# ekzhu/datasketch

Hardware: AMD Instinct MI355X
Metric: MinHash signatures/sec (1M sets x 256 tokens, num_perm=128) (higher is better)
Workload: dtype u64

## Files before the change

datasketch_amd/csrc/mhx_api.hip:

```cpp
#include <algorithm>
#include <cmath>
#include <condition_variable>
#include <cstdlib>
#include <cstring>
#include <mutex>
#include <new>
#include <system_error>
#include <thread>
#include <vector>

#include "mhx_internal.h"

namespace mhx {

static thread_local std::string g_last_error;

void set_error(const char *fmt, ...) {
    char buf[1024];
    va_list ap;
    va_start(ap, fmt);
    vsnprintf(buf, sizeof(buf), fmt, ap);
    va_end(ap);
    g_last_error = buf;
}
// ... 186 lines not shown
        (void)hipStreamSynchronize(stream);
        (void)mhx::dev_free(d_redo);
        d_redo = nullptr;
        redo_capacity = 0;
    }
    const int64_t cap = std::max<int64_t>(n_sets + n_sets / 4, 1024);
    hipError_t e = mhx::dev_malloc(reinterpret_cast<void **>(&d_redo), (size_t)cap + 64);
    if (e != hipSuccess) {
        d_redo = nullptr;
        return fail(MHX_ERR_OOM, "redo flag allocation of %lld bytes failed: %s", (long long)cap, hipGetErrorString(e));
    }
    redo_capacity = cap;
    return MHX_OK;
}

int mhx_ctx::ensure_work() {
    if (d_work) return MHX_OK;
    hipError_t e = mhx::dev_malloc(reinterpret_cast<void **>(&d_work), mhx::kWorkBytes);
    if (e != hipSuccess) {
        d_work = nullptr;
        return fail(MHX_ERR_OOM, "work counter allocation failed: %s", hipGetErrorString(e));
    }
    MHX_HIP_CHECK(hipMemsetAsync(d_work, 0, mhx::kWorkBytes, stream));
    return MHX_OK;
}

extern "C" {

const char *mhx_last_error(void) { return mhx::g_last_error.c_str(); }

const char *mhx_version(void) { return "mhx 0.1.0 (gfx950)"; }

int mhx_device_count(int *count) {
    if (!count) return fail(MHX_ERR_INVALID, "count is NULL");
    int n = 0;
    hipError_t e = hipGetDeviceCount(&n);
    if (e != hipSuccess) {
        (void)hipGetLastError();
        *count = 0;
        return MHX_OK;
    }
    *count = n;
    return MHX_OK;
}

int mhx_ctx_create(int device, mhx_ctx **out) {
// ... 12 lines not shown
    ctx->device = device;
    ctx->num_cus = prop.multiProcessorCount;
    ctx->lds_per_block = (int64_t)prop.sharedMemPerBlock;
    ctx->hbm_bytes = (int64_t)prop.totalGlobalMem;
    snprintf(ctx->name, sizeof(ctx->name), "%s (%s)", prop.name, prop.gcnArchName);
    hipError_t e = hipStreamCreateWithFlags(&ctx->stream, hipStreamNonBlocking);
    if (e != hipSuccess) {
        delete ctx;
        return fail(MHX_ERR_HIP, "hipStreamCreate failed: %s", hipGetErrorString(e));
    }
    *out = ctx;
    return MHX_OK;
}

int mhx_ctx_destroy(mhx_ctx *ctx) {
    if (!ctx) return MHX_OK;
    (void)hipSetDevice(ctx->device);
    (void)hipStreamSynchronize(ctx->stream);
    for (int i = 0; i < 5; ++i)
        if (ctx->scratch[i]) (void)mhx::dev_free(ctx->scratch[i]);
    if (ctx->d_stats) (void)mhx::dev_free(ctx->d_stats);
    if (ctx->d_redo) (void)mhx::dev_free(ctx->d_redo);
    if (ctx->d_work) (void)mhx::dev_free(ctx->d_work);
    if (ctx->copy_in) (void)hipStreamDestroy(ctx->copy_in);
    if (ctx->copy_out) (void)hipStreamDestroy(ctx->copy_out);
    (void)hipStreamDestroy(ctx->stream);
    delete ctx;
    return MHX_OK;
}

int mhx_ctx_synchronize(mhx_ctx *ctx) {
    if (!ctx) return fail(MHX_ERR_INVALID, "ctx is NULL");
    MHX_GUARD(ctx);
    MHX_HIP_CHECK(hipStreamSynchronize(ctx->stream));
    return MHX_OK;
}

int mhx_ctx_release_scratch(mhx_ctx *ctx) {
    if (!ctx) return fail(MHX_ERR_INVALID, "ctx is NULL");
    MHX_GUARD(ctx);
    if (int rc = ctx->activate()) return rc;
    MHX_HIP_CHECK(hipStreamSynchronize(ctx->stream));
    for (int i = 0; i < 5; ++i) {
        if (ctx->scratch[i]) MHX_HIP_CHECK(mhx::dev_free(ctx->scratch[i]));
        ctx->scratch[i] = nullptr;
        ctx->scratch_bytes[i] = 0;
// ... 5 lines not shown
    }
    return MHX_OK;
}

int mhx_ctx_device_info(mhx_ctx *ctx, char *name, int name_len, int *cus, int64_t *hbm_bytes) {
    if (!ctx) return fail(MHX_ERR_INVALID, "ctx is NULL");
    MHX_GUARD(ctx);
    if (name && name_len > 0) {
        strncpy(name, ctx->name, (size_t)name_len - 1);
        name[name_len - 1] = 0;
    }
    if (cus) *cus = ctx->num_cus;
    if (hbm_bytes) *hbm_bytes = ctx->hbm_bytes;
    return MHX_OK;
}

int mhx_ctx_set_option(mhx_ctx *ctx, const char *key, int64_t value) {
    if (!ctx || !key) return fail(MHX_ERR_INVALID, "ctx/key is NULL");
    MHX_GUARD(ctx);
    if (!strcmp(key, "minhash.path")) ctx->opt_minhash_path = value;
    else if (!strcmp(key, "minhash.split")) ctx->opt_minhash_split = value;
    else if (!strcmp(key, "minhash.packed")) ctx->opt_minhash_packed = value;
    else if (!strcmp(key, "minhash.ties")) ctx->opt_minhash_ties = value;
    else if (!strcmp(key, "minhash.p3")) ctx->opt_minhash_p3 = value;
    else if (!strcmp(key, "minhash.share")) ctx->opt_minhash_share = value;
    else if (!strcmp(key, "minhash.adapt")) ctx->opt_minhash_adapt = value;
    else if (!strcmp(key, "blocks_per_cu")) ctx->opt_blocks_per_cu = value;
    else if (!strcmp(key, "minhash.alias")) ctx->opt_minhash_alias = value;
    else if (!strcmp(key, "minhash.prefetch")) ctx->opt_minhash_prefetch = value;
    else if (!strcmp(key, "weighted.path")) ctx->opt_weighted_path = value;
    else if (!strcmp(key, "weighted.direct")) ctx->opt_weighted_direct = value;
    else if (!strcmp(key, "weighted.split")) ctx->opt_weighted_split = value;
    else if (!strcmp(key, "weighted.tail")) ctx->opt_weighted_tail = value;
    else if (!strcmp(key, "weighted.debug")) ctx->opt_weighted_debug = value;
    else if (!strcmp(key, "weighted.kernel")) ctx->opt_weighted_kernel = value;
    else if (!strcmp(key, "weighted.plan")) ctx->opt_weighted_plan = value;
    else if (!strcmp(key, "weighted.rescue")) ctx->opt_weighted_rescue = value;
    else if (!strcmp(key, "weighted.min_dim")) ctx->opt_weighted_min_dim = value;
    else if (!strcmp(key, "host.chunk_bytes")) ctx->opt_host_chunk_bytes = value;
    else if (!strcmp(key, "lsh.sort_bits")) ctx->opt_lsh_sort_bits = value;
    else if (!strcmp(key, "lsh.gather")) ctx->opt_lsh_gather = value;
    else if (!strcmp(key, "lsh.sort")) ctx->opt_lsh_sort = value;
    else if (!strcmp(key, "lsh.levels")) ctx->opt_lsh_levels = value;
    else if (!strcmp(key, "lsh.chunk")) ctx->opt_lsh_chunk = value;
    else if (!strcmp(key, "lsh.team")) ctx->opt_lsh_team = value;
    else if (!strcmp(key, "lsh.bigbins")) ctx->opt_lsh_bigbins = value;
    else if (!strcmp(key, "pack.fused")) ctx->opt_pack_fused = value;
    else if (!strcmp(key, "weighted.refill")) ctx->opt_weighted_refill = value;
    else if (!strcmp(key, "lsh.prehash")) ctx->opt_lsh_prehash = value;
    else if (!strcmp(key, "lsh.merge_items")) {
        if (value != 0 && value != 8 && value != 16) return fail(MHX_ERR_INVALID, "lsh.merge_items must be 0, 8 or 16");
        ctx->opt_lsh_merge_items = value;
    }
    else return fail(MHX_ERR_INVALID, "unknown option '%s'", key);
    return MHX_OK;
}

int mhx_ctx_minhash_mode(mhx_ctx *ctx, int reset, int *mode) {
    if (!ctx) return fail(MHX_ERR_INVALID, "ctx is NULL");
    MHX_GUARD(ctx);
    if (int rc = ctx->activate()) return rc;
    if (int rc = ctx->ensure_work()) return rc;
    unsigned int word = 0;
    MHX_HIP_CHECK(hipMemcpyAsync(&word, ctx->d_work + 8, sizeof(word), hipMemcpyDeviceToHost, ctx->stream));
    MHX_HIP_CHECK(hipStreamSynchronize(ctx->stream));
    if (mode) *mode = (int)word;
    if (reset) MHX_HIP_CHECK(hipMemsetAsync(ctx->d_work + 8, 0, sizeof(word), ctx->stream));
    return MHX_OK;
}

int mhx_ctx_minhash_flags(mhx_ctx *ctx, int64_t n_sets, uint8_t *flags) {
    if (!ctx) return fail(MHX_ERR_INVALID, "ctx is NULL");
    MHX_GUARD(ctx);
    if (int rc = ctx->activate()) return rc;
    MHX_REQUIRE(n_sets >= 0 && (flags || n_sets == 0), "NULL flags");
    if (ctx->redo_sets != n_sets || (n_sets > 0 && !ctx->d_redo))
        return fail(MHX_ERR_INVALID, "the last MinHash call on this context kept flags for %lld sets, not %lld (one huge set split over waves and "
                    "minhash.path != 0 keep none)", (long long)ctx->redo_sets, (long long)n_sets);
    MHX_HIP_CHECK(hipStreamSynchronize(ctx->stream));
    if (n_sets > 0) MHX_HIP_CHECK(hipMemcpy(flags, ctx->d_redo, (size_t)n_sets, hipMemcpyDeviceToHost));
    return MHX_OK;
}

int mhx_ctx_counters(mhx_ctx *ctx, int enable, uint64_t out[MHX_NUM_COUNTERS]) {
    if (!ctx) return fail(MHX_ERR_INVALID, "ctx is NULL");
    MHX_GUARD(ctx);
    if (int rc = ctx->activate()) return rc;
    MHX_HIP_CHECK(hipStreamSynchronize(ctx->stream));
    if (out) {
        for (int i = 0; i < MHX_NUM_COUNTERS; ++i) out[i] = 0;
// ... 1618 lines not shown
```

datasketch_amd/csrc/mhx_internal.h:

```cpp
#pragma once

#include <hip/hip_runtime.h>

#include <cstdarg>
#include <cstdint>
#include <cstdio>
#include <mutex>
#include <string>
#include <unordered_map>

#include "mhx.h"

namespace mhx {

void set_error(const char *fmt, ...);
int fail(int code, const char *fmt, ...);
void forgive();

#define MHX_HIP_CHECK(expr)                                                                      \
    do {                                                                                         \
        hipError_t _e = (expr);                                                                  \
        if (_e != hipSuccess) {                                                                  \
            return ::mhx::fail(_e == hipErrorOutOfMemory ? MHX_ERR_OOM : MHX_ERR_HIP,            \
                               "%s failed: %s (%s:%d)", #expr, hipGetErrorString(_e), __FILE__,  \
                               __LINE__);                                                        \
        }                                                                                        \
    } while (0)

constexpr int kSigDigests = 2;
constexpr int kSigDigestsBM = 3;

constexpr unsigned int kPairListCap = 16384;
constexpr size_t kWorkBytes = 64 + sizeof(unsigned int) * kPairListCap;

#define MHX_GUARD(ctxp) std::lock_guard<std::recursive_mutex> _mhx_guard((ctxp)->mu)

#define MHX_REQUIRE(cond, ...)                                       \
    do {                                                             \
        if (!(cond)) return ::mhx::fail(MHX_ERR_INVALID, __VA_ARGS__); \
    } while (0)

hipError_t dev_malloc(void **p, size_t bytes, bool caller = false);
hipError_t dev_free(void *p);
bool guard_mode();

}

struct mhx_ctx {
    std::recursive_mutex mu;
    int device = 0;
    hipStream_t stream = nullptr;
    int num_cus = 0;
    int64_t lds_per_block = 64 << 10;
    int64_t hbm_bytes = 0;
    char name[128] = {0};
    void *scratch[5] = {nullptr, nullptr, nullptr, nullptr, nullptr};
    size_t scratch_bytes[5] = {0, 0, 0, 0, 0};
    int64_t opt_minhash_path = 0;
    int64_t opt_minhash_packed = 0;
    int64_t opt_minhash_adapt = 0;
    int64_t opt_minhash_share = 0;
    int64_t opt_minhash_p3 = 0;
    int64_t opt_minhash_ties = 0;
    int64_t opt_minhash_split = 0;
    int64_t opt_blocks_per_cu = 0;
    int64_t opt_minhash_prefetch = 1;
    int64_t opt_minhash_alias = -1;
    int64_t opt_weighted_path = 0;
    int64_t opt_weighted_min_dim = 0;
    int64_t opt_weighted_rescue = 0;
    int64_t opt_weighted_plan = 0;
    int64_t opt_weighted_kernel = 0;
    int64_t opt_weighted_debug = 0;
    int64_t opt_weighted_split = 0;
    int64_t opt_weighted_tail = 0;
    int64_t opt_weighted_direct = 0;
    int64_t opt_lsh_sort = 0;
    int64_t opt_lsh_gather = 0;
    int64_t opt_lsh_sort_bits = 0;
    int64_t opt_lsh_prehash = 0;
    int64_t opt_lsh_chunk = 0;
    int64_t opt_lsh_bigbins = 0;
    int64_t opt_lsh_team = 0;
    int64_t opt_lsh_merge_items = 0;
    int64_t opt_lsh_levels = 0;
    int64_t opt_pack_fused = 0;
    int64_t opt_weighted_refill = 0;
    int64_t opt_host_chunk_bytes = 0;

    hipStream_t copy_in = nullptr;
    hipStream_t copy_out = nullptr;
    int ensure_copy_streams();

    unsigned long long *d_stats = nullptr;
    uint8_t *d_redo = nullptr;
    int64_t redo_capacity = 0;
    int64_t redo_sets = 0;
    int ensure_redo(int64_t n_sets);
    unsigned int *d_work = nullptr;
    int ensure_work();

    int ensure_scratch(int slot, size_t bytes);
    int activate() const;
};

struct mhx_perm {
    mhx_ctx *ctx = nullptr;
    int32_t num_perm = 0;
    uint64_t *d_a = nullptr;
    uint64_t *d_b = nullptr;
};

struct mhx_wgen {
    mhx_ctx *ctx = nullptr;
    int32_t sample_size = 0;
    int32_t dim = 0;
    float *d_params = nullptr;
    int32_t s_pad = 0;
    bool table_fast = false;
    float *d_aos = nullptr;
    float *d_walk_a = nullptr;
    uint32_t *d_walk_c = nullptr;
// ... 76 lines not shown
```

datasketch_amd/csrc/minhash_kernels.hip:

```cpp
#include <type_traits>

#include "mhx_internal.h"

namespace mhx {
namespace {

constexpr uint64_t kMersenne = (1ull << 61) - 1;
constexpr uint32_t kMaxHash = 0xFFFFFFFFu;
constexpr int kWave = 64;

struct BulkArgs {
    const void *hv;
    const int64_t *offsets;
    int64_t fixed_len;
    int64_t n_sets;
    const uint64_t *a;
    const uint64_t *b;
    int32_t num_perm;
    int32_t path;
    unsigned long long *stats;
    uint8_t *redo;
    int32_t redo_match;
    unsigned int *sieve_hint;
    unsigned int *mode_word;
    unsigned int *pair_count;
    unsigned int *pair_list;
    int32_t prefetch;
    int32_t ties;
    int32_t share_last;
    int64_t alias_mask;
    const uint64_t *init;
    int64_t init_stride;
    void *out;
};

__device__ __forceinline__ void mad_narrow(uint32_t h, uint32_t a_lo, uint32_t a_hi, uint64_t b,
                                           uint32_t &s_lo, uint32_t &s_hi) {
    const uint64_t s0 = (uint64_t)h * a_lo + b;
    s_lo = (uint32_t)s0;
    s_hi = (uint32_t)(s0 >> 32) + h * a_hi;
}

__device__ __forceinline__ void mad_wide(uint32_t h_lo, uint32_t h_hi, uint32_t a_lo, uint32_t a_hi,
                                         uint64_t b, uint32_t &s_lo, uint32_t &s_hi) {
    const uint64_t s0 = (uint64_t)h_lo * a_lo + b;
    s_lo = (uint32_t)s0;
    s_hi = (uint32_t)(s0 >> 32) + h_lo * a_hi + h_hi * a_lo;
// ... 694 lines not shown
        const int r = args.num_perm - (kbase + (P - 1) * kWave);
        span = r > 16 ? 32u : r > 8 ? 16u : r > 4 ? 8u : 4u;
    }
    sp.span = span;
#pragma unroll
    for (int p = 0; p < P; ++p) {
        const bool shared = SHARE && P >= 3 && p == P - 1;
        const int k = kbase + p * kWave + (shared ? lane & (int)(span - 1) : lane);
        const bool holds = k < args.num_perm;
        kidx[p] = holds && !(shared && lane >= (int)span) ? k : -1;
        const uint64_t a = holds ? args.a[k] : 0;
        pm.a_lo[p] = (uint32_t)a;
        pm.a_hi[p] = (uint32_t)(a >> 32);
        pm.b[p] = holds ? args.b[k] : 0;
        pm_biased.a_lo[p] = pm.a_lo[p];
        pm_biased.a_hi[p] = pm.a_hi[p];
        pm_biased.b[p] = pm.b[p] + 1;
        sp.a_lo[p] = pm.a_lo[p];
        sp.b8[p] = pm.b[p] + 8;
        sp.active[p] = kidx[p] >= 0;
    }
}

enum { MODE_SIEVE = 0, MODE_FULL = 1, MODE_DEDUP = 2, MODE_SIEVE_TIES = 3 };
enum { SHAPE_GENERAL = 0, SHAPE_PLAIN = 1, SHAPE_PLAIN_FIXED = 2, SHAPE_PLAIN_FIXED_ROWS = 3 };

template <int P, typename TokT, typename OutT, int MODE, int SHAPE, bool SHARE = false>
__global__ __launch_bounds__(256) void minhash_bulk_kernel(const BulkArgs args_in) {
    BulkArgs args = args_in;
    constexpr bool kSieve = MODE == MODE_SIEVE || MODE == MODE_SIEVE_TIES;
    if (kSieve && args.mode_word) {
        const unsigned int want_ties = *as_const(args.mode_word);
        if ((want_ties == 1u) != (MODE == MODE_SIEVE_TIES)) return;
    }
    if (MODE == MODE_FULL && args.mode_word && args.sieve_hint && blockIdx.x == 0 && threadIdx.x == 0) {
        const unsigned int t = __builtin_nontemporal_load(args.sieve_hint), f = __builtin_nontemporal_load(args.sieve_hint + 1);
        const unsigned int g = __builtin_nontemporal_load(args.sieve_hint + 2), m = *args.mode_word;
        const unsigned int tt = __builtin_nontemporal_load(args.sieve_hint + 3), tf = __builtin_nontemporal_load(args.sieve_hint + 5);
        if (t >= 64u) {
            const bool defeated = 4u * f > t;
            const bool heavy = m == 1u ? 5u * g > t : (tt >= 64u ? 5u * tf > tt : m == 2u);
            *args.mode_word = !defeated ? 0u : heavy ? 2u : 1u;
        }
    }
    if (SHAPE != SHAPE_GENERAL) {
        args.init = nullptr;
        args.init_stride = 0;
        args.stats = nullptr;
        args.alias_mask = -1;
    }
    if (SHAPE == SHAPE_PLAIN_FIXED || SHAPE == SHAPE_PLAIN_FIXED_ROWS) args.offsets = nullptr;
    const int lane = threadIdx.x & (kWave - 1);
    const int wave = __builtin_amdgcn_readfirstlane(threadIdx.x >> 6);
    const int waves_per_block = blockDim.x >> 6;
    const int kchunks = (args.num_perm + kWave * P - 1) / (kWave * P);
    constexpr int kLdsPerWave = MODE == MODE_DEDUP ? kDedupWordsPerWave : kStageWordsPerWave;
    __shared__ __attribute__((aligned(16))) uint32_t stage[4 * kLdsPerWave];
    uint32_t *lds = stage + wave * kLdsPerWave;
    Perms<P> pm, pm_biased;
    SievePerms<P> sp;
    int kidx[P];
    if (kSieve || MODE == MODE_DEDUP) load_perms<P, SHARE>(args, 0, lane, pm, pm_biased, sp, kidx);

    const TokT MHX_CONST_AS *hv = as_const(static_cast<const TokT *>(args.hv));
    const TokT *hv_vec = static_cast<const TokT *>(args.hv);
    const int64_t MHX_CONST_AS *offsets = as_const(args.offsets);
    OutT *__restrict__ out = static_cast<OutT *>(args.out);
    const int64_t stride = (int64_t)gridDim.x * waves_per_block;
    const bool flagged_only = !kSieve && args.redo != nullptr;
    unsigned int listed_n = 0;
    bool listed = false;
    if (MODE == MODE_FULL && flagged_only && args.pair_list) {
        listed_n = *as_const(args.pair_count);
        listed = listed_n <= kPairListCap;
    }
    const int64_t n_items = listed ? (int64_t)listed_n : flagged_only ? (args.n_sets + kWave - 1) / kWave * waves_per_block : args.n_sets;
    SieveBackoff backoff;
    TiesBackoff ties;
    int tried = 0, failed = 0, left = 0;
    if (MODE == MODE_SIEVE && args.sieve_hint) {
        const unsigned int t = __builtin_nontemporal_load(args.sieve_hint), f = __builtin_nontemporal_load(args.sieve_hint + 1);
        if (t >= 64u && 2u * f > t) {
            backoff.skip = 63;
            backoff.gap = 64;
            backoff.streak = 2;
        }
    }
    if (MODE == MODE_FULL && listed) {
        uint32_t *comb = stage;
        for (int64_t it = blockIdx.x; it < (int64_t)listed_n; it += gridDim.x) {
            const int64_t set = (int64_t)as_const(args.pair_list)[it];
            const int64_t beg = args.offsets ? offsets[set] : set * args.fixed_len;
            const int64_t end = args.offsets ? offsets[set + 1] : beg + args.fixed_len;
            const int64_t share = (end - beg + 31) / 32 * 8;
            const int64_t wbeg = min(end, beg + wave * share), wend = min(end, wbeg + share);
            for (int kc = 0; kc < kchunks; ++kc) {
                uint32_t mine[P];
#pragma unroll
                for (int p = 0; p < P; ++p) mine[p] = kMaxHash;
                if (wend > wbeg) {
                    const Minima<P> m = full_minima<P, TokT>(hv_vec, wbeg, wend, args.a, args.b, args.num_perm, kc * (kWave * P),
                                                             args.path == 1, args.stats);
#pragma unroll
                    for (int p = 0; p < P; ++p) mine[p] = m.v[p];
                }
#pragma unroll
                for (int p = 0; p < P; ++p) comb[(wave * P + p) * kWave + lane] = mine[p];
                __syncthreads();
                if (wave == 0) {
#pragma unroll
                    for (int p = 0; p < P; ++p) {
                        const int k = kc * (kWave * P) + p * kWave + lane;
                        if (k >= args.num_perm) continue;
                        uint32_t r = mine[p];
#pragma unroll
                        for (int w = 1; w < 4; ++w) r = min(r, comb[(w * P + p) * kWave + lane]);
                        uint64_t v = r;
                        if (args.init) {
                            const uint64_t iv = args.init[set * args.init_stride + k];
                            v = end > beg ? (uint64_t)min((iv >> 32) ? kMaxHash : (uint32_t)iv, r) : iv;
                        }
                        if (sizeof(OutT) == 4) v = v > kMaxHash ? kMaxHash : v;
                        out[set * args.num_perm + k] = (OutT)v;
                    }
                }
                __syncthreads();
            }
        }
        return;
    }
    for (int64_t item0 = (int64_t)blockIdx.x * waves_per_block + wave; item0 < n_items; item0 += stride) {
      const int64_t item = flagged_only ? item0 / waves_per_block : item0;
      unsigned long long todo = 1;
      if (flagged_only && !listed) {
          const int64_t cand = item * kWave + lane;
          const bool mine = (lane % waves_per_block) == (int)(item0 % waves_per_block);
          todo = __ballot(mine && cand < args.n_sets && args.redo[cand] == (uint8_t)args.redo_match);
      }
      while (todo) {
        const int bit = __builtin_ctzll(todo);
        todo &= todo - 1;
        const int64_t set = listed ? (int64_t)as_const(args.pair_list)[item0] : flagged_only ? item * kWave + bit : item;
        int64_t beg, end;
        if (args.offsets) {
            beg = offsets[set];
            end = offsets[set + 1];
        } else {
            beg = (args.alias_mask >= 0 ? (set & args.alias_mask) : set) * args.fixed_len;
            end = beg + args.fixed_len;
        }
        uint32_t warm = 0;
        {
            const int64_t nset = listed ? args.n_sets : flagged_only ? (todo ? item * kWave + __builtin_ctzll(todo) : args.n_sets) : item + stride;
            const bool skipping_on = MODE == MODE_SIEVE && backoff.skip > 1;
            if (args.prefetch && nset < args.n_sets && !skipping_on) {
                const int64_t nbeg = args.offsets ? offsets[nset] : nset * args.fixed_len;
                const int64_t nend = args.offsets ? offsets[nset + 1] : nbeg + args.fixed_len;
                const int64_t off = (int64_t)lane * 128;
                if (off < (nend - nbeg) * (int64_t)sizeof(TokT))
                    warm = *reinterpret_cast<const volatile uint32_t *>(reinterpret_cast<const char *>(args.hv) +
                                                                         nbeg * (int64_t)sizeof(TokT) + off);
            }
        }
        bool defer = false;
        if (MODE == MODE_SIEVE && end > beg && backoff.skip > 0) {
            --backoff.skip;
            defer = true;
        }
        for (int kc = 0; kc < kchunks && !defer; ++kc) {
            uint32_t res[P];
            if (kSieve) {
                if (kchunks > 1) load_perms<P, SHARE>(args, kc * (kWave * P), lane, pm, pm_biased, sp, kidx);
                if (end > beg) {
                    bool tied = false;
                    defer = sieve_minima<P, TokT, SHAPE != SHAPE_PLAIN_FIXED_ROWS, MODE == MODE_SIEVE_TIES, SHARE>(hv, hv_vec, beg, end, pm, pm_biased, sp, args.stats, lane, lds, res,
                                                                                                          MODE == MODE_SIEVE_TIES ? &tied : nullptr);
                    if (kc == 0) ++tried;
                    if (MODE == MODE_SIEVE_TIES) {
                        if (defer || __any(tied)) ++failed;
                        if (defer) {
                            ++left;
                            break;
                        }
                    } else {
                        if (defer) {
                            ++failed;
                            backoff.failed();
                            break;
                        }
                        backoff.succeeded();
// ... 39 lines not shown
#pragma unroll
            for (int p = 0; p < P; ++p) {
                if (kidx[p] < 0) continue;
                uint64_t v;
                if (args.init) {
                    const uint64_t iv = args.init[set * args.init_stride + kidx[p]];
                    if (end > beg) {
                        const uint32_t ic = (iv >> 32) ? kMaxHash : (uint32_t)iv;
                        v = min(ic, res[p]);
                    } else {
                        v = iv;
                    }
                } else {
                    v = end > beg ? res[p] : kMaxHash;
                }
                if (sizeof(OutT) == 4) v = v > kMaxHash ? kMaxHash : v;
                out[set * args.num_perm + kidx[p]] = (OutT)v;
            }
        }
        if (kSieve && lane == 0) {
            args.redo[set] = defer ? 1 : 0;
            if (defer && args.stats) atomicAdd(args.stats, 1ull);
        }
        if (MODE == MODE_DEDUP && defer && lane == 0) {
            args.redo[set] = 2;
            if (args.pair_list) {
                const unsigned int slot = atomicAdd(args.pair_count, 1u);
                if (slot < kPairListCap) args.pair_list[slot] = (unsigned int)set;
            }
        }
        asm volatile("" ::"v"(warm));
      }
    }
    if (kSieve && args.sieve_hint && lane == 0 && wave == 0 && (blockIdx.x & 15u) == 0 && tried > 0) {
        atomicAdd(args.sieve_hint, (unsigned int)tried);
        if (failed) atomicAdd(args.sieve_hint + 1, (unsigned int)failed);
        if (left) atomicAdd(args.sieve_hint + 2, (unsigned int)left);
    }
    if (MODE == MODE_DEDUP && args.sieve_hint && args.mode_word && lane == 0 && tried > 0) {
        atomicAdd(args.sieve_hint + 3, (unsigned int)tried);
        if (failed) atomicAdd(args.sieve_hint + 5, (unsigned int)failed);
    }
}

template <int KP, int P, typename TokT, typename OutT>
__global__ __launch_bounds__(256) void minhash_packed_kernel(const BulkArgs args) {
    constexpr int G = kWave / KP;
    constexpr int STRIDE = 36;
    const int lane = threadIdx.x & (kWave - 1);
    const int wave = __builtin_amdgcn_readfirstlane(threadIdx.x >> 6);
    const int g = lane / KP, k = lane % KP;
    __shared__ __attribute__((aligned(16))) uint32_t stage[4 * G * kStageWordsPerWave];
    uint32_t *tiles = stage + wave * (G * kStageWordsPerWave);
    uint32_t *my_tile = tiles + g * kStageWordsPerWave;
    Perms<P> pm;
    SievePerms<P> sp;
    bool any_active = false;
#pragma unroll
    for (int q = 0; q < P; ++q) {
        const bool active = k + q * KP < args.num_perm;
        const uint64_t a = active ? args.a[k + q * KP] : 0, b = active ? args.b[k + q * KP] : 0;
        pm.a_lo[q] = sp.a_lo[q] = (uint32_t)a;
        pm.a_hi[q] = (uint32_t)(a >> 32);
        pm.b[q] = b;
        sp.b8[q] = b + 8;
        sp.active[q] = active;
        any_active |= active;
    }
    const TokT *hv_vec = static_cast<const TokT *>(args.hv);
    OutT *__restrict__ out = static_cast<OutT *>(args.out);
    const unsigned long long group_lanes = (KP == 64 ? ~0ull : ((1ull << KP) - 1ull)) << (g * KP);
    const int64_t n_items = (args.n_sets + G - 1) / G;
    for (int64_t item = (int64_t)blockIdx.x * 4 + wave; item < n_items; item += (int64_t)gridDim.x * 4) {
        const int64_t set = item * G + g;
        const bool has = set < args.n_sets;
        int64_t beg = 0, end = 0;
        if (has) {
            beg = args.offsets ? args.offsets[set] : set * args.fixed_len;
            end = args.offsets ? args.offsets[set + 1] : beg + args.fixed_len;
        }
        uint32_t res[P];
#pragma unroll
        for (int q = 0; q < P; ++q) res[q] = kMaxHash;
        bool fail = false;
        for (int64_t boff = 0; __any(beg + boff < end); boff += kBlockRows * kRowTokens) {
            const int64_t blk = beg + boff;
            const int nb = (int)max((int64_t)0, min((int64_t)(kBlockRows * kRowTokens), end - blk));
#pragma unroll
            for (int j = 0; j < G; ++j) {
                const int jnb = __builtin_amdgcn_readlane(nb, j * KP);
                if (jnb == 0) continue;
                const uint32_t blo = __builtin_amdgcn_readlane((int)(uint32_t)blk, j * KP);
                const uint32_t bhi = __builtin_amdgcn_readlane((int)(uint32_t)((uint64_t)blk >> 32), j * KP);
                const int64_t jblk = (int64_t)(((uint64_t)bhi << 32) | blo);
                uint64_t t[4] = {0, 0, 0, 0};
// ... 41 lines not shown
#pragma unroll
                for (int q = 0; q < P; ++q) rows[q].add(r < nrows ? tag16(row[q], (uint32_t)r) : kMaxHash);
            }
            if (__any(rest > 0)) {
                uint32_t row[P];
#pragma unroll
                for (int q = 0; q < P; ++q) row[q] = kMaxHash;
                const uint32_t *rowp = my_tile + nrows * STRIDE;
                for (int c = 0; c < kRowTokens - 1; ++c) {
                    if (!__any(c < rest)) break;
                    const uint32_t h = rowp[2 * c];
#pragma unroll
                    for (int q = 0; q < P; ++q)
                        if (c < rest) row[q] = min(row[q], sieve_key(h, sp.a_lo[q], sp.b8[q]));
                }
#pragma unroll
                for (int q = 0; q < P; ++q)
                    if (rest > 0) rows[q].add(tag16(row[q], (uint32_t)nrows));
            }
            if (nb > 0) fail |= finish_block<P, STRIDE, 2, true>(rows, my_tile, pm, sp, res, (uint32_t)nrows, (uint32_t)rest);
        }
        const bool group_failed = (__ballot(fail && any_active) & group_lanes) != 0;
        if (has && k == 0) args.redo[set] = group_failed ? 1 : 0;
#pragma unroll
        for (int q = 0; q < P; ++q) {
            if (has && sp.active[q] && !group_failed) {
                uint64_t v;
                if (args.init) {
                    const uint64_t iv = args.init[set * args.init_stride + k + q * KP];
                    v = end > beg ? (uint64_t)min((iv >> 32) ? kMaxHash : (uint32_t)iv, res[q]) : iv;
                } else {
                    v = end > beg ? res[q] : kMaxHash;
                }
                if (sizeof(OutT) == 4) v = v > kMaxHash ? kMaxHash : v;
                out[set * args.num_perm + k + q * KP] = (OutT)v;
            }
        }
    }
}

template <typename OutT>
__global__ void minhash_fill_state_kernel(const BulkArgs args) {
    const int64_t total = args.n_sets * (int64_t)args.num_perm;
    OutT *__restrict__ out = static_cast<OutT *>(args.out);
    for (int64_t i = (int64_t)blockIdx.x * blockDim.x + threadIdx.x; i < total;
         i += (int64_t)gridDim.x * blockDim.x) {
        uint64_t v = kMaxHash;
        if (args.init) {
            const int64_t set = i / args.num_perm;
            v = args.init[set * args.init_stride + (i - set * args.num_perm)];
        }
        if (sizeof(OutT) == 4) v = v > kMaxHash ? kMaxHash : v;
        out[i] = (OutT)v;
    }
}

template <int P, typename TokT, typename OutT>
__global__ __launch_bounds__(256) void minhash_split_kernel(const BulkArgs args, int64_t first_token,
                                                            int64_t total_tokens, int64_t slice) {
    const int lane = threadIdx.x & (kWave - 1);
    const int wave = __builtin_amdgcn_readfirstlane(threadIdx.x >> 6);
// ... 78 lines not shown
    if ((count & 1) && blockIdx.x == 0 && threadIdx.x == 0)
        out[count - 1] = x[count - 1] < y[count - 1] ? x[count - 1] : y[count - 1];
}

unsigned resident_grid(mhx_ctx *ctx, const void *kernel, int64_t items) {
    int per_cu = 0;
    if (hipOccupancyMaxActiveBlocksPerMultiprocessor(&per_cu, kernel, 256, 0) != hipSuccess || per_cu < 1) {
        (void)hipGetLastError();
        per_cu = 2;
    }
    return (unsigned)std::max<int64_t>(1, std::min<int64_t>(items, (int64_t)ctx->num_cus * per_cu));
}

template <int P, typename TokT, typename OutT, int PF = P>
int launch_typed(mhx_ctx *ctx, const BulkArgs &args, int64_t first_token, int64_t total_tokens, bool split) {
    const int kchunks = (args.num_perm + kWave * P - 1) / (kWave * P);
    const int blocks_per_cu = ctx->opt_blocks_per_cu > 0 ? (int)ctx->opt_blocks_per_cu : (P >= 3 ? 128 : 64);
    const int64_t max_blocks = (int64_t)ctx->num_cus * blocks_per_cu;
    if (!split) {
        const int64_t want = (args.n_sets + 3) / 4;
        dim3 grid((unsigned)std::max<int64_t>(1, std::min(want, max_blocks)), 1u);
        if (args.path == 0) {
            if (int rc = ctx->ensure_work()) return rc;
            MHX_HIP_CHECK(hipMemsetAsync(ctx->d_work, 0, 8 * sizeof(unsigned int), ctx->stream));
            BulkArgs sieve_args = args;
            sieve_args.sieve_hint = ctx->d_work;
            sieve_args.mode_word = ctx->opt_minhash_adapt == 1 || args.stats ? nullptr : ctx->d_work + 8;
            const BulkArgs &args_s = sieve_args;
            const bool plain = !args.init && !args.stats && args.alias_mask < 0;
            const int np = args.num_perm;
            const bool packable = !args.stats && args.alias_mask < 0 && ctx->opt_minhash_packed != 1;
            const bool packed = packable && P <= 2 && (np <= 96 || (ctx->opt_minhash_packed == 2 && np <= 128));
            if (packed) {
                const int kp = np <= 8 ? 8 : np <= 16 ? 16 : np <= 32 ? 32 : np <= 64 ? 16 : np <= 96 ? 32 : 64;
                const int64_t items = (args.n_sets + 64 / kp - 1) / (64 / kp);
                dim3 pgrid((unsigned)std::max<int64_t>(1, std::min<int64_t>((items + 3) / 4, max_blocks)), 1u);
#define MHX_PACKED(KP_, P_) hipLaunchKernelGGL((minhash_packed_kernel<KP_, P_, TokT, OutT>), pgrid, dim3(256), 0, ctx->stream, args_s)
                if (np <= 8) MHX_PACKED(8, 1);
                else if (np <= 16) MHX_PACKED(16, 1);
                else if (np <= 32) MHX_PACKED(32, 1);
                else if (np <= 48) MHX_PACKED(16, 3);
                else if (np <= 64) MHX_PACKED(16, 4);
                else if (np <= 96) MHX_PACKED(32, 3);
                else MHX_PACKED(64, 2);
#undef MHX_PACKED
            } else {
            const bool fixed_rows = plain && !args.offsets && args.fixed_len % kRowTokens == 0;
            const int last_slot = args.num_perm - (P - 1) * kWave;
            const bool share = P >= 3 && kchunks == 1 && args.share_last && last_slot > 0 && last_slot <= 32;
            const auto first_launches = [&](auto share_tag) {
                constexpr bool SH = decltype(share_tag)::value;
#define MHX_SIEVE(MODE_, SHAPE_) hipLaunchKernelGGL((minhash_bulk_kernel<P, TokT, OutT, MODE_, SHAPE_, SH>), grid, dim3(256), 0, ctx->stream, args_s)
                if (fixed_rows) MHX_SIEVE(MODE_SIEVE, SHAPE_PLAIN_FIXED_ROWS);
                else if (plain && !args.offsets) MHX_SIEVE(MODE_SIEVE, SHAPE_PLAIN_FIXED);
                else if (plain) MHX_SIEVE(MODE_SIEVE, SHAPE_PLAIN);
                else MHX_SIEVE(MODE_SIEVE, SHAPE_GENERAL);
                if (args_s.mode_word) {
                    if (fixed_rows) MHX_SIEVE(MODE_SIEVE_TIES, SHAPE_PLAIN_FIXED_ROWS);
                    else MHX_SIEVE(MODE_SIEVE_TIES, SHAPE_GENERAL);
                }
#undef MHX_SIEVE
            };
            if constexpr (P >= 3) {
                if (share) first_launches(std::true_type());
                else first_launches(std::false_type());
            } else {
                (void)share;
                first_launches(std::false_type());
            }
            }
            const int64_t flag_groups = (args.n_sets + kWave - 1) / kWave;
            BulkArgs dedup = args;
            dedup.redo_match = 1;
            dedup.sieve_hint = sieve_args.sieve_hint;
            dedup.mode_word = packed ? nullptr : sieve_args.mode_word;
            if (args.n_sets <= 0xFFFFFFFFll) {
                dedup.pair_count = ctx->d_work + 4;
                dedup.pair_list = ctx->d_work + 16;
            }
            hipLaunchKernelGGL((minhash_bulk_kernel<PF, TokT, OutT, MODE_DEDUP, SHAPE_GENERAL>),
                               dim3(resident_grid(ctx, (const void *)minhash_bulk_kernel<PF, TokT, OutT, MODE_DEDUP, SHAPE_GENERAL>, flag_groups)),
                               dim3(256), 0, ctx->stream, dedup);
            BulkArgs rest = dedup;
            rest.redo_match = 2;
            hipLaunchKernelGGL((minhash_bulk_kernel<PF, TokT, OutT, MODE_FULL, SHAPE_GENERAL>),
                               dim3(resident_grid(ctx, (const void *)minhash_bulk_kernel<PF, TokT, OutT, MODE_FULL, SHAPE_GENERAL>, flag_groups)),
                               dim3(256), 0, ctx->stream, rest);
        } else {
            BulkArgs all = args;
            all.redo = nullptr;
            hipLaunchKernelGGL((minhash_bulk_kernel<PF, TokT, OutT, MODE_FULL, SHAPE_GENERAL>), grid, dim3(256), 0, ctx->stream, all);
        }
    } else {
        const int64_t total_out = args.n_sets * (int64_t)args.num_perm;
        const int64_t fill_blocks = std::max<int64_t>(1, std::min<int64_t>((total_out + 255) / 256, max_blocks));
        hipLaunchKernelGGL((minhash_fill_state_kernel<OutT>), dim3((unsigned)fill_blocks), dim3(256), 0,
                           ctx->stream, args);
        const int64_t waves = (int64_t)ctx->num_cus * 32;
// ... 24 lines not shown

}

int launch_minhash_bulk(mhx_perm *perm, const void *d_hv, int hv_dtype, const int64_t *d_offsets,
                        int64_t fixed_len, int64_t n_sets, int64_t total_tokens,
                        const uint64_t *d_init, int64_t init_stride, void *d_out, int out_dtype, int64_t first_token) {
    mhx_ctx *ctx = perm->ctx;
    if (n_sets == 0) return MHX_OK;
    total_tokens -= first_token;
    BulkArgs args;
    args.hv = d_hv;
    args.offsets = d_offsets;
    args.fixed_len = fixed_len;
    args.n_sets = n_sets;
    args.a = perm->d_a;
    args.b = perm->d_b;
    args.num_perm = perm->num_perm;
    args.path = (int32_t)ctx->opt_minhash_path;
    args.stats = ctx->d_stats;
    args.redo = nullptr;
    args.redo_match = 1;
    args.sieve_hint = nullptr;
    args.mode_word = nullptr;
    args.alias_mask = ctx->opt_minhash_alias;
    args.pair_count = nullptr;
    args.pair_list = nullptr;
    args.prefetch = ctx->opt_minhash_prefetch == 2 || (ctx->opt_minhash_prefetch == 1 && (d_offsets != nullptr || fixed_len < 256));
    args.ties = ctx->opt_minhash_ties != 1;
    args.share_last = ctx->opt_minhash_share != 1;
    args.init = d_init;
    args.init_stride = init_stride;
    args.out = d_out;
    const int64_t waves_avail = (int64_t)ctx->num_cus * 16;
    bool split = n_sets < waves_avail && total_tokens > n_sets * 128 && total_tokens >= 1024;
    if (ctx->opt_minhash_split == 1) split = false;
    if (ctx->opt_minhash_split == 2) split = total_tokens > 0;
    ctx->redo_sets = 0;
    if (!split && args.path == 0) {
        if (int rc = ctx->ensure_redo(n_sets)) return rc;
        args.redo = ctx->d_redo;
        ctx->redo_sets = n_sets;
    }
    if (hv_dtype == MHX_U64 && out_dtype == MHX_U64) return launch_p<uint64_t, uint64_t>(ctx, args, first_token, total_tokens, split);
    if (hv_dtype == MHX_U64 && out_dtype == MHX_U32) return launch_p<uint64_t, uint32_t>(ctx, args, first_token, total_tokens, split);
    if (hv_dtype == MHX_U32 && out_dtype == MHX_U64) return launch_p<uint32_t, uint64_t>(ctx, args, first_token, total_tokens, split);
    if (hv_dtype == MHX_U32 && out_dtype == MHX_U32) return launch_p<uint32_t, uint32_t>(ctx, args, first_token, total_tokens, split);
// ... 16 lines not shown
```

Baseline: 496.3 million.

## Replace dedup+full redo passes with single compact redo-list kernel

Sieve kernels now append deferred set indices to a bounded redo list in the work buffer. A new redo kernel settles only the listed sets, doing the ties, dedup and pairwise fallback in one launch, and replaces the separate dedup and full-grid passes. When the list overflows, it falls back to scanning the per-set redo flags. The last block writes mode and overflow state to host-mapped memory so the next call can skip the plain sieve launch and choose ties-first without a host sync, which adds grid-wide atomics and a dependency on the previous call's state.

Result: slower. 487.0 million (-1.9%).

```diff
diff --git a/datasketch_amd/csrc/mhx_api.hip b/datasketch_amd/csrc/mhx_api.hip
--- a/datasketch_amd/csrc/mhx_api.hip
+++ b/datasketch_amd/csrc/mhx_api.hip
@@ -232,6 +232,17 @@
         return fail(MHX_ERR_OOM, "work counter allocation failed: %s", hipGetErrorString(e));
     }
     MHX_HIP_CHECK(hipMemsetAsync(d_work, 0, mhx::kWorkBytes, stream));
+    if (!h_plan) {
+        void *h = nullptr, *d = nullptr;
+        MHX_HIP_CHECK(hipHostMalloc(&h, 64, hipHostMallocMapped | hipHostMallocCoherent));
+        if (hipError_t e2 = hipHostGetDevicePointer(&d, h, 0); e2 != hipSuccess) {
+            (void)hipHostFree(h);
+            return fail(MHX_ERR_HIP, "hipHostGetDevicePointer failed: %s", hipGetErrorString(e2));
+        }
+        memset(h, 0, 64);
+        h_plan = static_cast<volatile unsigned int *>(h);
+        d_plan = static_cast<unsigned int *>(d);
+    }
     return MHX_OK;
 }
 
@@ -290,6 +301,7 @@
     if (ctx->d_stats) (void)mhx::dev_free(ctx->d_stats);
     if (ctx->d_redo) (void)mhx::dev_free(ctx->d_redo);
     if (ctx->d_work) (void)mhx::dev_free(ctx->d_work);
+    if (ctx->h_plan) (void)hipHostFree(const_cast<unsigned int *>(ctx->h_plan));
     if (ctx->copy_in) (void)hipStreamDestroy(ctx->copy_in);
     if (ctx->copy_out) (void)hipStreamDestroy(ctx->copy_out);
     (void)hipStreamDestroy(ctx->stream);
@@ -341,6 +353,7 @@
     else if (!strcmp(key, "minhash.split")) ctx->opt_minhash_split = value;
     else if (!strcmp(key, "minhash.packed")) ctx->opt_minhash_packed = value;
     else if (!strcmp(key, "minhash.ties")) ctx->opt_minhash_ties = value;
+    else if (!strcmp(key, "minhash.redo")) ctx->opt_minhash_redo = value;
     else if (!strcmp(key, "minhash.p3")) ctx->opt_minhash_p3 = value;
     else if (!strcmp(key, "minhash.share")) ctx->opt_minhash_share = value;
     else if (!strcmp(key, "minhash.adapt")) ctx->opt_minhash_adapt = value;
@@ -384,7 +397,10 @@
     MHX_HIP_CHECK(hipMemcpyAsync(&word, ctx->d_work + 8, sizeof(word), hipMemcpyDeviceToHost, ctx->stream));
     MHX_HIP_CHECK(hipStreamSynchronize(ctx->stream));
     if (mode) *mode = (int)word;
-    if (reset) MHX_HIP_CHECK(hipMemsetAsync(ctx->d_work + 8, 0, sizeof(word), ctx->stream));
+    if (reset) {
+        MHX_HIP_CHECK(hipMemsetAsync(ctx->d_work + mhx::kWorkMode, 0, sizeof(word), ctx->stream));
+        ctx->h_plan[0] = ctx->h_plan[1] = 0;
+    }
     return MHX_OK;
 }
 
diff --git a/datasketch_amd/csrc/mhx_internal.h b/datasketch_amd/csrc/mhx_internal.h
--- a/datasketch_amd/csrc/mhx_internal.h
+++ b/datasketch_amd/csrc/mhx_internal.h
@@ -31,7 +31,10 @@
 constexpr int kSigDigestsBM = 3;
 
 constexpr unsigned int kPairListCap = 16384;
-constexpr size_t kWorkBytes = 64 + sizeof(unsigned int) * kPairListCap;
+constexpr unsigned int kRedoListCap = 4096;
+constexpr int kWorkRedoCount = 6, kWorkOverflow = 7, kWorkMode = 8, kWorkDone = 9;
+constexpr int kWorkPairList = 16, kWorkRedoList = kWorkPairList + (int)kPairListCap;
+constexpr size_t kWorkBytes = sizeof(unsigned int) * (kWorkRedoList + kRedoListCap);
 
 #define MHX_GUARD(ctxp) std::lock_guard<std::recursive_mutex> _mhx_guard((ctxp)->mu)
 
@@ -62,6 +65,7 @@
     int64_t opt_minhash_share = 0;
     int64_t opt_minhash_p3 = 0;
     int64_t opt_minhash_ties = 0;
+    int64_t opt_minhash_redo = 0;
     int64_t opt_minhash_split = 0;
     int64_t opt_blocks_per_cu = 0;
     int64_t opt_minhash_prefetch = 1;
@@ -98,6 +102,8 @@
     int64_t redo_sets = 0;
     int ensure_redo(int64_t n_sets);
     unsigned int *d_work = nullptr;
+    volatile unsigned int *h_plan = nullptr;
+    unsigned int *d_plan = nullptr;
     int ensure_work();
 
     int ensure_scratch(int slot, size_t bytes);
diff --git a/datasketch_amd/csrc/minhash_kernels.hip b/datasketch_amd/csrc/minhash_kernels.hip
--- a/datasketch_amd/csrc/minhash_kernels.hip
+++ b/datasketch_amd/csrc/minhash_kernels.hip
@@ -23,6 +23,9 @@
     int32_t redo_match;
     unsigned int *sieve_hint;
     unsigned int *mode_word;
+    unsigned int *obey_word;
+    unsigned int *plan;
+    int32_t first_ties;
     unsigned int *pair_count;
     unsigned int *pair_list;
     int32_t prefetch;
@@ -763,6 +766,97 @@
     }
 }
 
+__device__ __forceinline__ void learn_mode(unsigned int *work, unsigned int *mode_word, bool ran_ties) {
+    const unsigned int t = atomicAdd(work, 0u), f = atomicAdd(work + 1, 0u), g = atomicAdd(work + 2, 0u);
+    const unsigned int tt = atomicAdd(work + 3, 0u), tf = atomicAdd(work + 5, 0u);
+    if (t >= 64u) {
+        const bool defeated = 4u * f > t;
+        const bool heavy = ran_ties ? 5u * g > t : (tt >= 64u ? 5u * tf > tt : *mode_word == 2u);
+        *mode_word = !defeated ? 0u : heavy ? 2u : 1u;
+    }
+}
+
+__device__ __forceinline__ void close_call(const BulkArgs &args, bool learn, bool ran_ties) {
+    unsigned int *work = args.sieve_hint;
+    __threadfence();
+    if (atomicAdd(work + kWorkDone, 1u) != gridDim.x - 1u) return;
+    __threadfence();
+    if (learn && args.mode_word) learn_mode(work, args.mode_word, ran_ties);
+    if (args.plan) {
+        args.plan[0] = atomicAdd(work + kWorkMode, 0u);
+        args.plan[1] = (atomicAdd(work + kWorkOverflow, 0u) != 0u || atomicAdd(work + kWorkRedoCount, 0u) > kRedoListCap) ? 1u : 0u;
+        __threadfence_system();
+    }
+#pragma unroll
+    for (int i = 0; i < 8; ++i) work[i] = 0u;
+    work[kWorkDone] = 0u;
+}
+
+struct RedoList {
+    unsigned int closed = 1u;
+    __device__ __forceinline__ void open(unsigned int *work) {
+        closed = work == nullptr ? 1u : (unsigned int)__builtin_amdgcn_readfirstlane((int)__builtin_nontemporal_load(work + kWorkOverflow));
+    }
+    __device__ __forceinline__ void overflow(unsigned int *work, int lane) {
+        if (closed) return;
+        if (lane == 0) work[kWorkOverflow] = 1u;
+        closed = 1u;
+    }
+    __device__ __forceinline__ void defer(unsigned int *work, int64_t set, int lane) {
+        if (closed) return;
+        unsigned int slot = 0;
+        if (lane == 0) slot = atomicAdd(work + kWorkRedoCount, 1u);
+        slot = (unsigned int)__builtin_amdgcn_readfirstlane((int)slot);
+        if (slot < kRedoListCap) {
+            if (lane == 0) work[kWorkRedoList + slot] = (unsigned int)set;
+        } else {
+            overflow(work, lane);
+        }
+    }
+};
+
+template <int P, typename TokT, typename OutT>
+__device__ __forceinline__ void pairwise_set(const BulkArgs &args, int64_t set, int64_t beg, int64_t end, uint32_t *comb, int lane,
+                                             int wave) {
+    const TokT *hv_vec = static_cast<const TokT *>(args.hv);
+    OutT *__restrict__ out = static_cast<OutT *>(args.out);
+    const int kchunks = (args.num_perm + kWave * P - 1) / (kWave * P);
+    const int64_t share = (end - beg + 31) / 32 * 8;
+    const int64_t wbeg = min(end, beg + wave * share), wend = min(end, wbeg + share);
+    for (int kc = 0; kc < kchunks; ++kc) {
+        uint32_t mine[P];
+#pragma unroll
+        for (int p = 0; p < P; ++p) mine[p] = kMaxHash;
+        if (wend > wbeg) {
+            const Minima<P> m = full_minima<P, TokT>(hv_vec, wbeg, wend, args.a, args.b, args.num_perm, kc * (kWave * P),
+                                                     args.path == 1, args.stats);
+#pragma unroll
+            for (int p = 0; p < P; ++p) mine[p] = m.v[p];
+        }
+#pragma unroll
+        for (int p = 0; p < P; ++p) comb[(wave * P + p) * kWave + lane] = mine[p];
+        __syncthreads();
+        if (wave == 0) {
+#pragma unroll
+            for (int p = 0; p < P; ++p) {
+                const int k = kc * (kWave * P) + p * kWave + lane;
+                if (k >= args.num_perm) continue;
+                uint32_t r = mine[p];
+#pragma unroll
+                for (int w = 1; w < 4; ++w) r = min(r, comb[(w * P + p) * kWave + lane]);
+                uint64_t v = r;
+                if (args.init) {
+                    const uint64_t iv = args.init[set * args.init_stride + k];
+                    v = end > beg ? (uint64_t)min((iv >> 32) ? kMaxHash : (uint32_t)iv, r) : iv;
+                }
+                if (sizeof(OutT) == 4) v = v > kMaxHash ? kMaxHash : v;
+                out[set * args.num_perm + k] = (OutT)v;
+            }
+        }
+        __syncthreads();
+    }
+}
+
 enum { MODE_SIEVE = 0, MODE_FULL = 1, MODE_DEDUP = 2, MODE_SIEVE_TIES = 3 };
 enum { SHAPE_GENERAL = 0, SHAPE_PLAIN = 1, SHAPE_PLAIN_FIXED = 2, SHAPE_PLAIN_FIXED_ROWS = 3 };
 
@@ -770,20 +864,12 @@
 __global__ __launch_bounds__(256) void minhash_bulk_kernel(const BulkArgs args_in) {
     BulkArgs args = args_in;
     constexpr bool kSieve = MODE == MODE_SIEVE || MODE == MODE_SIEVE_TIES;
-    if (kSieve && args.mode_word) {
-        const unsigned int want_ties = *as_const(args.mode_word);
+    if (kSieve && args.obey_word) {
+        const unsigned int want_ties = *as_const(args.obey_word);
         if ((want_ties == 1u) != (MODE == MODE_SIEVE_TIES)) return;
     }
-    if (MODE == MODE_FULL && args.mode_word && args.sieve_hint && blockIdx.x == 0 && threadIdx.x == 0) {
-        const unsigned int t = __builtin_nontemporal_load(args.sieve_hint), f = __builtin_nontemporal_load(args.sieve_hint + 1);
-        const unsigned int g = __builtin_nontemporal_load(args.sieve_hint + 2), m = *args.mode_word;
-        const unsigned int tt = __builtin_nontemporal_load(args.sieve_hint + 3), tf = __builtin_nontemporal_load(args.sieve_hint + 5);
-        if (t >= 64u) {
-            const bool defeated = 4u * f > t;
-            const bool heavy = m == 1u ? 5u * g > t : (tt >= 64u ? 5u * tf > tt : m == 2u);
-            *args.mode_word = !defeated ? 0u : heavy ? 2u : 1u;
-        }
-    }
+    if (MODE == MODE_FULL && args.mode_word && args.sieve_hint && blockIdx.x == 0 && threadIdx.x == 0)
+        learn_mode(args.sieve_hint, args.mode_word, *args.mode_word == 1u);
     if (SHAPE != SHAPE_GENERAL) {
         args.init = nullptr;
         args.init_stride = 0;
@@ -819,6 +905,8 @@
     SieveBackoff backoff;
     TiesBackoff ties;
     int tried = 0, failed = 0, left = 0;
+    RedoList redo_list;
+    if (kSieve) redo_list.open(args.sieve_hint);
     if (MODE == MODE_SIEVE && args.sieve_hint) {
         const unsigned int t = __builtin_nontemporal_load(args.sieve_hint), f = __builtin_nontemporal_load(args.sieve_hint + 1);
         if (t >= 64u && 2u * f > t) {
@@ -828,46 +916,14 @@
         }
     }
     if (MODE == MODE_FULL && listed) {
-        uint32_t *comb = stage;
         for (int64_t it = blockIdx.x; it < (int64_t)listed_n; it += gridDim.x) {
             const int64_t set = (int64_t)as_const(args.pair_list)[it];
             const int64_t beg = args.offsets ? offsets[set] : set * args.fixed_len;
             const int64_t end = args.offsets ? offsets[set + 1] : beg + args.fixed_len;
-            const int64_t share = (end - beg + 31) / 32 * 8;
-            const int64_t wbeg = min(end, beg + wave * share), wend = min(end, wbeg + share);
-            for (int kc = 0; kc < kchunks; ++kc) {
-                uint32_t mine[P];
-#pragma unroll
-                for (int p = 0; p < P; ++p) mine[p] = kMaxHash;
-                if (wend > wbeg) {
-                    const Minima<P> m = full_minima<P, TokT>(hv_vec, wbeg, wend, args.a, args.b, args.num_perm, kc * (kWave * P),
-                                                             args.path == 1, args.stats);
-#pragma unroll
-                    for (int p = 0; p < P; ++p) mine[p] = m.v[p];
-                }
-#pragma unroll
-                for (int p = 0; p < P; ++p) comb[(wave * P + p) * kWave + lane] = mine[p];
-                __syncthreads();
-                if (wave == 0) {
-#pragma unroll
-                    for (int p = 0; p < P; ++p) {
-                        const int k = kc * (kWave * P) + p * kWave + lane;
-                        if (k >= args.num_perm) continue;
-                        uint32_t r = mine[p];
-#pragma unroll
-                        for (int w = 1; w < 4; ++w) r = min(r, comb[(w * P + p) * kWave + lane]);
-                        uint64_t v = r;
-                        if (args.init) {
-                            const uint64_t iv = args.init[set * args.init_stride + k];
-                            v = end > beg ? (uint64_t)min((iv >> 32) ? kMaxHash : (uint32_t)iv, r) : iv;
-                        }
-                        if (sizeof(OutT) == 4) v = v > kMaxHash ? kMaxHash : v;
-                        out[set * args.num_perm + k] = (OutT)v;
-                    }
-                }
-                __syncthreads();
-            }
-        }
+            pairwise_set<P, TokT, OutT>(args, set, beg, end, stage, lane, wave);
+        }
+        __syncthreads();
+        if (threadIdx.x == 0 && args.sieve_hint) close_call(args, false, false);
         return;
     }
     for (int64_t item0 = (int64_t)blockIdx.x * waves_per_block + wave; item0 < n_items; item0 += stride) {
@@ -907,6 +963,7 @@
         if (MODE == MODE_SIEVE && end > beg && backoff.skip > 0) {
             --backoff.skip;
             defer = true;
+            redo_list.overflow(args.sieve_hint, lane);
         }
         for (int kc = 0; kc < kchunks && !defer; ++kc) {
             uint32_t res[P];
@@ -992,6 +1049,7 @@
             args.redo[set] = defer ? 1 : 0;
             if (defer && args.stats) atomicAdd(args.stats, 1ull);
         }
+        if (kSieve && defer) redo_list.defer(args.sieve_hint, set, lane);
         if (MODE == MODE_DEDUP && defer && lane == 0) {
             args.redo[set] = 2;
             if (args.pair_list) {
@@ -1010,6 +1068,10 @@
     if (MODE == MODE_DEDUP && args.sieve_hint && args.mode_word && lane == 0 && tried > 0) {
         atomicAdd(args.sieve_hint + 3, (unsigned int)tried);
         if (failed) atomicAdd(args.sieve_hint + 5, (unsigned int)failed);
+    }
+    if (MODE == MODE_FULL && flagged_only && args.sieve_hint) {
+        __syncthreads();
+        if (threadIdx.x == 0) close_call(args, false, false);
     }
 }
 
@@ -1041,6 +1103,9 @@
     OutT *__restrict__ out = static_cast<OutT *>(args.out);
     const unsigned long long group_lanes = (KP == 64 ? ~0ull : ((1ull << KP) - 1ull)) << (g * KP);
     const int64_t n_items = (args.n_sets + G - 1) / G;
+    unsigned int *work = args.sieve_hint;
+    RedoList redo_list;
+    redo_list.open(work);
     for (int64_t item = (int64_t)blockIdx.x * 4 + wave; item < n_items; item += (int64_t)gridDim.x * 4) {
         const int64_t set = item * G + g;
         const bool has = set < args.n_sets;
@@ -1128,6 +1193,19 @@
         }
         const bool group_failed = (__ballot(fail && any_active) & group_lanes) != 0;
         if (has && k == 0) args.redo[set] = group_failed ? 1 : 0;
+        const bool hand_over = has && k == 0 && group_failed;
+        if (redo_list.closed == 0u && __any(hand_over)) {
+            bool over = false;
+            if (hand_over) {
+                const unsigned int slot = atomicAdd(work + kWorkRedoCount, 1u);
+                if (slot < kRedoListCap) work[kWorkRedoList + slot] = (unsigned int)set;
+                else over = true;
+            }
+            if (__any(over)) {
+                if (lane == 0) work[kWorkOverflow] = 1u;
+                redo_list.closed = 1u;
+            }
+        }
 #pragma unroll
         for (int q = 0; q < P; ++q) {
             if (has && sp.active[q] && !group_failed) {
@@ -1143,6 +1221,171 @@
             }
         }
     }
+}
+
+template <int P, typename TokT, typename OutT>
+__global__ __launch_bounds__(256) void minhash_redo_kernel(const BulkArgs args) {
+    constexpr int STRIDE = 36;
+    const int tid = threadIdx.x, lane = tid & (kWave - 1);
+    const int wave = __builtin_amdgcn_readfirstlane(tid >> 6);
+    const int kchunks = (args.num_perm + kWave * P - 1) / (kWave * P);
+    __shared__ __attribute__((aligned(16))) uint32_t tile[kStageWordsPerWave];
+    __shared__ __attribute__((aligned(16))) uint32_t priv[4 * kDedupWordsPerWave];
+    __shared__ unsigned long long s_mask[4];
+    __shared__ unsigned int s_pair;
+    unsigned int *work = args.sieve_hint;
+    const TokT *hv_vec = static_cast<const TokT *>(args.hv);
+    const int64_t MHX_CONST_AS *offsets = as_const(args.offsets);
+    OutT *__restrict__ out = static_cast<OutT *>(args.out);
+    const bool try_ties = args.ties && !args.first_ties;
+    TiesBackoff ties;
+    int tried = 0, failed = 0;
+
+    const auto settle = [&](int64_t set) {
+        int64_t beg, end;
+        if (args.offsets) {
+            beg = offsets[set];
+            end = offsets[set + 1];
+        } else {
+            beg = (args.alias_mask >= 0 ? (set & args.alias_mask) : set) * args.fixed_len;
+            end = beg + args.fixed_len;
+        }
+        __syncthreads();
+        if (tid == 0) s_pair = 0u;
+        for (int kc0 = 0; kc0 < kchunks; kc0 += 4) {
+            const int kc = kc0 + wave;
+            const bool mine = kc < kchunks;
+            Perms<P> pm, pm_biased;
+            SievePerms<P> sp;
+            int kidx[P];
+            load_perms<P>(args, (mine ? kc : 0) * (kWave * P), lane, pm, pm_biased, sp, kidx);
+            uint32_t res[P];
+#pragma unroll
+            for (int p = 0; p < P; ++p) res[p] = kMaxHash;
+            bool with_ties = mine && try_ties;
+            if (with_ties && ties.skip > 0) {
+                --ties.skip;
+                with_ties = false;
+            }
+            bool fail = false;
+            for (int64_t blk = beg; blk < end; blk += kBlockRows * kRowTokens) {
+                const int nb = (int)min((int64_t)(kBlockRows * kRowTokens), end - blk);
+                __syncthreads();
+                if (tid < nb) {
+                    const uint64_t t = (uint64_t)hv_vec[blk + tid];
+                    uint32_t *cell = tile + (tid >> 4) * STRIDE + (tid & 15) * 2;
+                    cell[0] = (uint32_t)t;
+                    cell[1] = (uint32_t)(t >> 32);
+                }
+                __syncthreads();
+                if (!with_ties) continue;
+                const int nrows = nb >> 4;
+                Three rows[P];
+                for (int r = 0; r < nrows; ++r) {
+                    const uint4 *rowq = reinterpret_cast<const uint4 *>(tile + r * STRIDE);
+                    uint32_t row[P];
+#pragma unroll
+                    for (int half = 0; half < 2; ++half) {
+                        uint4 two[4];
+#pragma unroll
+                        for (int c2 = 0; c2 < 4; ++c2) two[c2] = rowq[4 * half + c2];
+#pragma unroll
+                        for (int c2 = 0; c2 < 4; ++c2) {
+#pragma unroll
+                            for (int q = 0; q < P; ++q) {
+                                const uint32_t k0 = sieve_key(two[c2].x, sp.a_lo[q], sp.b8[q]);
+                                const uint32_t k1 = sieve_key(two[c2].z, sp.a_lo[q], sp.b8[q]);
+                                row[q] = (half == 0 && c2 == 0) ? min(k0, k1) : umin3(row[q], k0, k1);
+                            }
+                        }
+                        __builtin_amdgcn_sched_barrier(0);
+                    }
+#pragma unroll
+                    for (int q = 0; q < P; ++q) rows[q].add(tag16(row[q], (uint32_t)r));
+                }
+                if (nrows > 0) fail |= finish_block_ties<P, STRIDE, 2>(rows, tile, pm, sp, res);
+                for (int c = nrows * kRowTokens; c < nb; ++c) {
+                    const uint32_t *cell = tile + (c >> 4) * STRIDE + (c & 15) * 2;
+                    const uint32_t lo = cell[0], hi = cell[1];
+#pragma unroll
+                    for (int q = 0; q < P; ++q) {
+                        uint32_t l0, h0;
+                        mad_wide(lo, hi, pm.a_lo[q], pm.a_hi[q], pm.b[q], l0, h0);
+                        res[q] = min(res[q], fold_exact(l0, h0));
+                    }
+                }
+            }
+            bool open = mine;
+            if (with_ties) {
+                open = __any(fail);
+                if (kc == 0) ++tried, failed += open ? 1 : 0;
+                if (open) ties.failed(); else ties.succeeded();
+            }
+            bool pair = false;
+            if (open && end > beg) {
+#pragma unroll
+                for (int p = 0; p < P; ++p) res[p] = kMaxHash;
+                uint64_t cur[4];
+                load_quad<TokT>(hv_vec, beg, end, lane, cur);
+                pair = __any(dedup_sieve_range<P, TokT>(hv_vec, beg, end, pm, sp, priv + wave * kDedupWordsPerWave, lane, cur, res));
+                if (pair && lane == 0) s_pair = 1u;
+            }
+            if (mine && !pair) {
+#pragma unroll
+                for (int p = 0; p < P; ++p) {
+                    if (kidx[p] < 0) continue;
+                    uint64_t v;
+                    if (args.init) {
+                        const uint64_t iv = args.init[set * args.init_stride + kidx[p]];
+                        v = end > beg ? (uint64_t)min((iv >> 32) ? kMaxHash : (uint32_t)iv, res[p]) : iv;
+                    } else {
+                        v = end > beg ? res[p] : kMaxHash;
+                    }
+                    if (sizeof(OutT) == 4) v = v > kMaxHash ? kMaxHash : v;
+                    out[set * args.num_perm + kidx[p]] = (OutT)v;
+                }
+            }
+        }
+        __syncthreads();
+        if (s_pair != 0u) {
+            if (tid == 0) {
+                args.redo[set] = 2;
+                if (args.stats) atomicAdd(args.stats + 3, 1ull);
+            }
+            pairwise_set<P, TokT, OutT>(args, set, beg, end, priv, lane, wave);
+        }
+    };
+
+    const unsigned int listed_n = *as_const(work + kWorkRedoCount);
+    const bool overflow = *as_const(work + kWorkOverflow) != 0u || listed_n > kRedoListCap;
+    if (!overflow) {
+        for (unsigned int it = blockIdx.x; it < listed_n; it += gridDim.x) settle((int64_t)as_const(work + kWorkRedoList)[it]);
+    } else {
+        const int64_t groups = (args.n_sets + 255) / 256;
+        for (int64_t g = blockIdx.x; g < groups; g += gridDim.x) {
+            const int64_t cand = g * 256 + tid;
+            const unsigned long long m = __ballot(cand < args.n_sets && args.redo[cand] == (uint8_t)1);
+            __syncthreads();
+            if (lane == 0) s_mask[wave] = m;
+            __syncthreads();
+            for (int w = 0; w < 4; ++w) {
+                const unsigned long long mw = s_mask[w];
+                unsigned long long todo = ((unsigned long long)(uint32_t)__builtin_amdgcn_readfirstlane((int)(uint32_t)(mw >> 32)) << 32) |
+                                          (uint32_t)__builtin_amdgcn_readfirstlane((int)(uint32_t)mw);
+                while (todo) {
+                    const int bit = __builtin_ctzll(todo);
+                    todo &= todo - 1;
+                    settle(g * 256 + w * kWave + bit);
+                }
+            }
+        }
+    }
+    if (args.mode_word && lane == 0 && tried > 0) {
+        atomicAdd(work + 3, (unsigned int)tried);
+        if (failed) atomicAdd(work + 5, (unsigned int)failed);
+    }
+    __syncthreads();
+    if (tid == 0) close_call(args, true, args.first_ties != 0);
 }
 
 template <typename OutT>
@@ -1267,10 +1510,14 @@
         dim3 grid((unsigned)std::max<int64_t>(1, std::min(want, max_blocks)), 1u);
         if (args.path == 0) {
             if (int rc = ctx->ensure_work()) return rc;
-            MHX_HIP_CHECK(hipMemsetAsync(ctx->d_work, 0, 8 * sizeof(unsigned int), ctx->stream));
+            const unsigned int seen_mode = ctx->h_plan[0], seen_overflow = ctx->h_plan[1];
+            const bool plan_a = ctx->opt_minhash_redo != 1 && seen_overflow == 0 && args.n_sets <= 0xFFFFFFFFll;
             BulkArgs sieve_args = args;
             sieve_args.sieve_hint = ctx->d_work;
-            sieve_args.mode_word = ctx->opt_minhash_adapt == 1 || args.stats ? nullptr : ctx->d_work + 8;
+            sieve_args.plan = ctx->d_plan;
+            sieve_args.mode_word = ctx->opt_minhash_adapt == 1 || args.stats ? nullptr : ctx->d_work + kWorkMode;
+            sieve_args.obey_word = plan_a ? nullptr : sieve_args.mode_word;
+            const bool ties_first = plan_a && sieve_args.mode_word && seen_mode == 1u;
             const BulkArgs &args_s = sieve_args;
             const bool plain = !args.init && !args.stats && args.alias_mask < 0;
             const int np = args.num_perm;
@@ -1296,11 +1543,12 @@
             const auto first_launches = [&](auto share_tag) {
                 constexpr bool SH = decltype(share_tag)::value;
 #define MHX_SIEVE(MODE_, SHAPE_) hipLaunchKernelGGL((minhash_bulk_kernel<P, TokT, OutT, MODE_, SHAPE_, SH>), grid, dim3(256), 0, ctx->stream, args_s)
-                if (fixed_rows) MHX_SIEVE(MODE_SIEVE, SHAPE_PLAIN_FIXED_ROWS);
+                if (ties_first) {
+                } else if (fixed_rows) MHX_SIEVE(MODE_SIEVE, SHAPE_PLAIN_FIXED_ROWS);
                 else if (plain && !args.offsets) MHX_SIEVE(MODE_SIEVE, SHAPE_PLAIN_FIXED);
                 else if (plain) MHX_SIEVE(MODE_SIEVE, SHAPE_PLAIN);
                 else MHX_SIEVE(MODE_SIEVE, SHAPE_GENERAL);
-                if (args_s.mode_word) {
+                if (plan_a ? ties_first : args_s.mode_word != nullptr) {
                     if (fixed_rows) MHX_SIEVE(MODE_SIEVE_TIES, SHAPE_PLAIN_FIXED_ROWS);
                     else MHX_SIEVE(MODE_SIEVE_TIES, SHAPE_GENERAL);
                 }
@@ -1315,10 +1563,17 @@
             }
             }
             const int64_t flag_groups = (args.n_sets + kWave - 1) / kWave;
-            BulkArgs dedup = args;
+            BulkArgs dedup = sieve_args;
             dedup.redo_match = 1;
-            dedup.sieve_hint = sieve_args.sieve_hint;
+            dedup.obey_word = nullptr;
             dedup.mode_word = packed ? nullptr : sieve_args.mode_word;
+            if (plan_a) {
+                dedup.first_ties = ties_first && !packed ? 1 : 0;
+                const unsigned rgrid = (unsigned)std::max<int64_t>(1, std::min<int64_t>(kRedoListCap, (int64_t)ctx->num_cus * 2));
+                hipLaunchKernelGGL((minhash_redo_kernel<PF, TokT, OutT>), dim3(rgrid), dim3(256), 0, ctx->stream, dedup);
+                MHX_HIP_CHECK(hipGetLastError());
+                return MHX_OK;
+            }
             if (args.n_sets <= 0xFFFFFFFFll) {
                 dedup.pair_count = ctx->d_work + 4;
                 dedup.pair_list = ctx->d_work + 16;
@@ -1389,6 +1644,9 @@
     args.redo_match = 1;
     args.sieve_hint = nullptr;
     args.mode_word = nullptr;
+    args.obey_word = nullptr;
+    args.plan = nullptr;
+    args.first_ties = 0;
     args.alias_mask = ctx->opt_minhash_alias;
     args.pair_count = nullptr;
     args.pair_list = nullptr;
```
